# jts/nanopolish

Hardware: NVIDIA H100
Metric: hmm_scored_events_per_sec (higher is better)
Workload: dtype f32

## Files before the change

### nanopolish_b200/csrc/hmm_classes.h

```cpp
#pragma once
#include <stdint.h>

#ifdef __CUDACC__
#define NPH_HD __host__ __device__ __forceinline__
#else
#define NPH_HD inline
#endif

#define NPH_NUM_WIDTHS 5
#define NPH_MAX_COLS 10
#define NPH_NUM_CLASSES (NPH_NUM_WIDTHS * NPH_MAX_COLS)
#define NPH_STEP_BUCKETS 1024
#define NPH_CHUNK_BUCKETS 8
#define NPH_KEY_BUCKETS (NPH_STEP_BUCKETS * NPH_CHUNK_BUCKETS)
#define NPH_MIN_PERIOD 40

NPH_HD uint32_t nph_class_width(int wi) { return wi >= 3 ? 32u : (4u << wi); }
NPH_HD bool nph_class_chained(int wi) { return wi == 4; }
NPH_HD int nph_class_index(int C, int wi) { return wi * NPH_MAX_COLS + (C - 1); }

NPH_HD uint32_t nph_class_steps(uint32_t K, uint32_t E, int C, uint32_t W)
{
    const uint32_t strip = W * (uint32_t)C;
    const uint32_t n_strips = (K + strip - 1) / strip;
    const uint32_t P = n_strips > 1 ? (E > (uint32_t)NPH_MIN_PERIOD ? E : (uint32_t)NPH_MIN_PERIOD) : E;
    const uint32_t last_cols = K - (n_strips - 1) * strip;
    return (n_strips - 1) * P + E + (last_cols - 1) / (uint32_t)C;
}

NPH_HD float nph_class_cost(uint32_t steps, int C, uint32_t W)
{
    return (float)steps * (46.0f + 67.0f * C) * (W * (1.0f / 32.0f));
}

NPH_HD int nph_choose_class(uint32_t K, uint32_t E, uint32_t* steps_out)
{
    float best = 3.0e38f;
    int best_cls = nph_class_index(NPH_MAX_COLS, 4);
    uint32_t best_steps = 0;
    for (int wi = 0; wi < NPH_NUM_WIDTHS; ++wi) {
        const uint32_t W = nph_class_width(wi);
        for (int C = 1; C <= NPH_MAX_COLS; ++C) {
            const bool fits = K <= W * (uint32_t)C;
            if (nph_class_chained(wi) ? fits : !fits) continue;
            const uint32_t steps = nph_class_steps(K, E, C, W);
            const float cost = nph_class_cost(steps, C, W);
            if (cost < best) { best = cost; best_cls = nph_class_index(C, wi); best_steps = steps; }
        }
    }
    *steps_out = best_steps;
    return best_cls;
}

NPH_HD uint32_t nph_key_bucket(uint32_t steps, uint32_t chunk)
{
    uint32_t b = steps < 768u ? steps : 768u + (steps - 768u) / 32u;
    if (b >= (uint32_t)NPH_STEP_BUCKETS) b = (uint32_t)NPH_STEP_BUCKETS - 1u;
    if (chunk >= (uint32_t)NPH_CHUNK_BUCKETS) chunk = (uint32_t)NPH_CHUNK_BUCKETS - 1u;
    return chunk * (uint32_t)NPH_STEP_BUCKETS + ((uint32_t)NPH_STEP_BUCKETS - 1u - b);
}
```

### nanopolish_b200/csrc/hmm_forward.cu

```cuda
#include "hmm_forward_kernel.cuh"
#include <algorithm>
#include <cmath>
#include <vector>

using namespace nph_fwd;

namespace {

__global__ void read_prologue_kernel(const DevRead* __restrict__ reads, const double* __restrict__ drift,
                                     const float* __restrict__ ev_mean, const double* __restrict__ ev_time,
                                     float* __restrict__ level, uint32_t n_reads)
{
    for (uint32_t r = blockIdx.x; r < n_reads; r += gridDim.x) {
        const DevRead rd = reads[r];
        const double dr = drift[r];
        const float* m = ev_mean + rd.event_off;
        const double* t = ev_time + rd.event_off;
        float* out = level + rd.event_off;
        const double t0 = t[0];
        for (uint32_t i = threadIdx.x; i < rd.n_events; i += blockDim.x) {
            const float time = (float)__dsub_rn(t[i], t0);
            out[i] = (float)__dsub_rn((double)m[i], __dmul_rn((double)time, dr));
        }
    }
}

}

static void scratch_layout(const nph_ctx* ctx, NphArena& a, float4** params, float** edge)
{
    const size_t warps = (size_t)ctx->sm_count * kMaxWarpsPerCta;
    for (int si = 0; si < nph_ctx::kSideStreams; ++si) {
        params[si] = a.take<float4>((size_t)ctx->max_kpad * warps);
        edge[si] = a.take<float>(3 * ((size_t)ctx->max_period + 8) * warps);
    }
}

size_t nph_hmm_scratch_bytes(const nph_ctx* ctx)
{
    float4* params[nph_ctx::kSideStreams];
    float* edge[nph_ctx::kSideStreams];
    return nph_layout_bytes([&](NphArena& a) { scratch_layout(ctx, a, params, edge); });
}

int nph_launch_read_prologue(nph_ctx* ctx)
{
    const uint32_t n = (uint32_t)ctx->n_reads;
    if (n == 0) return NPH_OK;
    int grid = (int)std::min<size_t>(n, (size_t)ctx->sm_count * 16);
    read_prologue_kernel<<<grid, 256, 0, ctx->stream>>>(ctx->d_reads.p, ctx->d_drift.p, ctx->d_ev_mean.p,
                                                        ctx->d_ev_time.p, ctx->d_level.p, n);
    NPH_CUDA(ctx, cudaGetLastError());
    return NPH_OK;
}

int nph_launch_hmm_forward(nph_ctx* ctx, float* scores_dev)
{
    FwdParams p{};
    p.level = ctx->d_level.p;
    p.reads = ctx->d_reads.p;
    p.trans = ctx->d_trans.p;
    p.models = ctx->d_models.p;
    p.ranks = ctx->d_ranks.p;
    p.jobs = ctx->d_jobs.p;
    p.logsum_g = ctx->d_logsum.p;
    p.flank = ctx->d_flank.p;
    p.scores = scores_dev ? scores_dev : ctx->d_scores.p;
    p.kpad_stride = ctx->max_kpad;
    p.edge_stride = ctx->max_period + 8;
    p.c = ctx->consts;
    p.lsum_bias = NPH_LOGSUM_SAT_ADDR_BIAS;
    p.lsum_scale = 4u;
    p.progress = (ctx->levels_inflight && ctx->level_chunk_events) ? ctx->d_progress.p : nullptr;
    p.chunk_events = (uint32_t)ctx->level_chunk_events;
    float4* params[nph_ctx::kSideStreams];
    float* edge[nph_ctx::kSideStreams];
    NphArena scratch{ctx->d_scratch.p};
    scratch_layout(ctx, scratch, params, edge);

    NPH_CUDA(ctx, cudaMemsetAsync(ctx->d_counters.p, 0, sizeof(unsigned int) * NPH_NUM_COUNTERS, ctx->stream));
    NPH_CUDA(ctx, cudaEventRecord(ctx->ev0, ctx->stream));
    NPH_CUDA(ctx, cudaEventRecord(ctx->ev_fork, ctx->stream));
    std::vector<size_t> idx;
    for (size_t ci = 0; ci < ctx->classes.size(); ++ci) if (ctx->classes[ci].count) idx.push_back(ci);
    std::sort(idx.begin(), idx.end(), [&](size_t a, size_t b) { return ctx->classes[a].cost > ctx->classes[b].cost; });
    bool used[nph_ctx::kSideStreams] = {false, false, false, false};
    int launches = 0;
    for (size_t t = 0; t < idx.size(); ++t) {
        const size_t ci = idx[t];
        const auto& cl = ctx->classes[ci];
        const int si = (int)(t % nph_ctx::kSideStreams);
        cudaStream_t st = ctx->side[si];
        if (!used[si]) { NPH_CUDA(ctx, cudaStreamWaitEvent(st, ctx->ev_fork, 0)); used[si] = true; }
        p.scratch_params = params[si];
        p.scratch_edge = edge[si];
        int rc = NPH_ERR_STATE;
        switch (cl.group_width) {
            case 4: rc = launch_width<4, false>(ctx, p, cl, (int)ci, st); break;
            case 8: rc = launch_width<8, false>(ctx, p, cl, (int)ci, st); break;
            case 16: rc = launch_width<16, false>(ctx, p, cl, (int)ci, st); break;
            case 32: rc = cl.chained ? launch_width<32, true>(ctx, p, cl, (int)ci, st) : launch_width<32, false>(ctx, p, cl, (int)ci, st); break;
        }
        if (rc != NPH_OK) return rc;
        ++launches;
    }
    for (int si = 0; si < nph_ctx::kSideStreams; ++si) {
        if (!used[si]) continue;
        NPH_CUDA(ctx, cudaEventRecord(ctx->ev_join[si], ctx->side[si]));
        NPH_CUDA(ctx, cudaStreamWaitEvent(ctx->stream, ctx->ev_join[si], 0));
    }
    NPH_CUDA(ctx, cudaEventRecord(ctx->ev1, ctx->stream));
    nph_timing_events(ctx, launches);
    return NPH_OK;
}
```

### nanopolish_b200/csrc/hmm_forward_kernel.cuh

```cuda
#pragma once
#include "nph_internal.cuh"
#include "hmm_classes.h"
#include "exact_math.cuh"
#include <math_constants.h>
#include <climits>

namespace nph_fwd {

static_assert(NPH_TBL_SMEM == NPH_LOGSUM_TBL_LEN, "the shared table must cover every index lsum_sat can form");

constexpr int kMaxWarpsPerCta = 24;
template <int C, int W> struct CtaShape { static constexpr int warps = (W == 32) ? 16 : (C <= 4 ? 24 : (C <= 6 ? 20 : 16)); };
constexpr unsigned kFull = 0xffffffffu;

struct FwdParams {
    const float* level;
    const DevRead* reads;
    const float2* trans;
    const DevModelView* models;
    const uint32_t* ranks;
    const nph_hmm_job* jobs;
    const uint32_t* order;
    uint32_t n_jobs;
    unsigned int* counter;
    const float* logsum_g;
    const float* flank;
    float* scores;
    float4* scratch_params;
    float* scratch_edge;
    uint32_t kpad_stride;
    uint32_t edge_stride;
    uint32_t lsum_bias;
    uint32_t lsum_scale;
    const uint32_t* progress;
    uint32_t chunk_events;
    HmmConsts c;
};

template <int C, int W, bool CHAIN>
__global__ void __launch_bounds__(CtaShape<C, W>::warps * 32, 1) hmm_forward_kernel(const FwdParams p)
{
    static_assert(W == 4 || W == 8 || W == 16 || W == 32, "group width");
    static_assert(!CHAIN || W == 32, "only full-warp groups chain strips");
    constexpr int G = 32 / W;
    constexpr int kWarpsPerCta = CtaShape<C, W>::warps;
    constexpr int kCtaThreads = kWarpsPerCta * 32;
    constexpr int STRIP = W * C;
    extern __shared__ float s_tbl[];
    for (int i = threadIdx.x; i < NPH_TBL_SMEM; i += kCtaThreads) s_tbl[i] = p.logsum_g[i];
    __syncthreads();
    const LogsumTable tb = make_logsum_table(s_tbl, p.lsum_bias, p.lsum_scale);

    const int lane = threadIdx.x & 31;
    const int gl = lane & (W - 1);
    const int grp = lane / W;
    const int warp_global = blockIdx.x * kWarpsPerCta + (threadIdx.x >> 5);
    float4* const my_params = p.scratch_params + (size_t)warp_global * p.kpad_stride + (W < 32 ? grp * STRIP : 0);
    float* const edge_m = p.scratch_edge + (size_t)warp_global * 3 * p.edge_stride;
    float* const edge_t = edge_m + p.edge_stride;
    float* const edge_k = edge_t + p.edge_stride;

    const float NEG = -CUDART_INF_F;
    const float lp_mk = p.c.lp_mk, lp_mb = p.c.lp_mb, lp_bb = p.c.lp_bb, lp3 = p.c.lp_bk;
    const float lp_kk = p.c.lp_kk, lp_km = p.c.lp_km;

    for (;;) {
        uint32_t base = 0;
        if (lane == 0) base = atomicAdd(p.counter, (unsigned)G);
        base = __shfl_sync(kFull, base, 0);
        if (base >= p.n_jobs) break;
        const uint32_t slot = base + grp;
        const bool has_job = slot < p.n_jobs;
        const uint32_t job_idx = p.order[has_job ? slot : base];
        const nph_hmm_job job = p.jobs[job_idx];
        const DevRead rd = p.reads[job.read];
        const float2 tr = p.trans[job.read];
        const float lp_mm_self = tr.x, lp_mm_next = tr.y;
        const DevModelView mv = p.models[job.model_id];
        if (p.progress) {
            uint32_t need = has_job ? (uint32_t)((rd.event_off + rd.n_events - 1) / p.chunk_events) + 1u : 0u;
            need = __reduce_max_sync(kFull, need);
            if (lane == 0) {
                const volatile uint32_t* pr = p.progress;
                while (*pr < need) __nanosleep(500);
            }
            __syncwarp();
        }

        const int K = (int)job.n_kmers;
        const int E = has_job ? (int)(job.event_stop > job.event_start ? job.event_stop - job.event_start
                                                                       : job.event_start - job.event_stop) + 1
                              : 0;
        const int stride = job.stride;
        const bool pre_clip = (job.flags & NPH_HAF_ALLOW_PRE_CLIP) != 0;
        const bool post_clip = (job.flags & NPH_HAF_ALLOW_POST_CLIP) != 0;
        const int n_strips = CHAIN ? (K + STRIP - 1) / STRIP : 1;
        const int kpad = n_strips * STRIP;
        const int P = n_strips > 1 ? max(E, NPH_MIN_PERIOD) : E;

        if (has_job) {
            const uint32_t* rk = p.ranks + job.rank_off;
            for (int i = gl; i < kpad; i += W) {
                float4 g = make_float4(0.f, 1.f, 0.f, 1.f);
                if (i < K) g = nph_scaled_gaussian(mv, rd, rk[i], p.c.log_inv_sqrt_2pi);
                my_params[i] = g;
            }
        }
        __syncwarp();

        const float* lv = p.level + rd.event_off;
        const long long e_first = (long long)job.event_start;

        const int last_strip = n_strips - 1;
        const int last_rel = (K - 1) - last_strip * STRIP;
        const int end_lane = last_rel / C;
        const int end_slot = last_rel % C;
        const int my_steps = has_job ? last_strip * P + E + end_lane : 0;
        const int total_steps = (W == 32) ? my_steps : __reduce_max_sync(kFull, my_steps);
        const bool any_pre_clip = __any_sync(kFull, pre_clip);

        float mu[C], sd[C], cc[C], ry[C];
        float Mp[C], Bp[C], Kp[C], Tp[C];
#pragma unroll
        for (int c = 0; c < C; ++c) { mu[c] = 0.f; sd[c] = 1.f; cc[c] = 0.f; ry[c] = 1.f; Mp[c] = NEG; Bp[c] = NEG; Kp[c] = NEG; Tp[c] = NEG; }
        if (!CHAIN && gl * C < K) {
#pragma unroll
            for (int c = 0; c < C; ++c) {
                const float4 g4 = my_params[gl * C + c];
                mu[c] = g4.x; sd[c] = g4.y; cc[c] = g4.z; ry[c] = g4.w;
            }
        }
        float Lm_prev = NEG, Lt_prev = NEG, Lk_prev = NEG;
        float lp_end = NEG;
        int r = 1 - gl;
        int s = 0;
        float x_next = 0.f;
        if (r == 1 && E >= 1) x_next = lv[e_first];
        float em_next = NEG, et_next = NEG, ek_next = NEG;
        const long long x_step = (long long)stride * (long long)sizeof(float);
        unsigned long long x_addr = (unsigned long long)(lv + e_first) + (unsigned long long)((long long)r * x_step);
        const int end_row = (gl == end_lane) ? (post_clip ? 1 : E) : INT_MAX;

        for (int g = 0; g < total_steps; ++g) {
            float Lm = __shfl_up_sync(kFull, Mp[C - 1], 1, W);
            float Lt = __shfl_up_sync(kFull, Tp[C - 1], 1, W);
            float Lk = __shfl_up_sync(kFull, Kp[C - 1], 1, W);
            if (gl == 0) { Lm = CHAIN ? em_next : NEG; Lt = CHAIN ? et_next : NEG; Lk = CHAIN ? ek_next : NEG; }

            const bool in_strip = (r >= 1) && (!CHAIN || s < n_strips);
            const int col0 = (CHAIN ? s * STRIP : 0) + gl * C;
            const bool live = in_strip && (r <= E) && (col0 < K);
            const float x = x_next;

            if (CHAIN && in_strip && r == 1) {
#pragma unroll
                for (int c = 0; c < C; ++c) { Mp[c] = NEG; Bp[c] = NEG; Kp[c] = NEG; Tp[c] = NEG; }
                Lm_prev = NEG; Lt_prev = NEG; Lk_prev = NEG;
                if (col0 < K) {
#pragma unroll
                    for (int c = 0; c < C; ++c) {
                        const float4 g4 = my_params[col0 + c];
                        mu[c] = g4.x; sd[c] = g4.y; cc[c] = g4.z; ry[c] = g4.w;
                    }
                }
            }

            {
                int rn = r + 1, sn = s;
                if (CHAIN && rn > P) { rn = 1; sn = s + 1; }
                if (rn >= 1 && rn <= E && (!CHAIN || sn < n_strips)) {
                    x_next = CHAIN ? lv[e_first + (long long)(rn - 1) * stride] : __ldca(reinterpret_cast<const float*>(x_addr));
                    if (CHAIN && gl == 0 && sn > 0) { em_next = edge_m[rn]; et_next = edge_t[rn]; ek_next = edge_k[rn]; }
                }
            }

            if (live) {
                const bool do_end = (!CHAIN || s == last_strip) && r >= end_row;

                float lm_prev = Lm_prev, lt_prev = Lt_prev, lk_prev = Lk_prev;
                float lm_cur = Lm, lt_cur = Lt, lk_cur = Lk;
                auto cell = [&](const int c, const bool with_soft) {
                    const float a = div_by_cached_rcp(__fsub_rn(x, mu[c]), sd[c], ry[c]);
                    const float em = add_neg_half_square(cc[c], a);
                    float m = __fadd_rn(lp_mm_self, Mp[c]);
                    m = lsum_sat(m, __fadd_rn(lp_mm_next, lm_prev), tb);
                    m = lsum_sat(m, Tp[c], tb);
                    m = lsum_sat(m, lt_prev, tb);
                    m = lsum_sat(m, __fadd_rn(lp_km, lk_prev), tb);
                    if (with_soft) m = lsum_sat(m, (col0 == 0 && (r == 1 || pre_clip)) ? p.flank[r - 1] : NEG, tb);
                    m = __fadd_rn(m, em);
                    const float b = lsum_sat(__fadd_rn(lp_mb, Mp[c]), __fadd_rn(lp_bb, Bp[c]), tb);
                    float kk = lsum_sat(__fadd_rn(lp_mk, lm_cur), lt_cur, tb);
                    kk = lsum_sat(kk, __fadd_rn(lp_kk, lk_cur), tb);
                    const float t = __fadd_rn(lp3, b);

                    lm_prev = Mp[c]; lt_prev = Tp[c]; lk_prev = Kp[c];
                    lm_cur = m; lt_cur = t; lk_cur = kk;
                    Mp[c] = m; Bp[c] = b; Kp[c] = kk; Tp[c] = t;
                };
                if (any_pre_clip || g == 0) cell(0, true);
                else cell(0, false);
#pragma unroll
                for (int c = 1; c < C; ++c) cell(c, false);
                Lm_prev = Lm; Lt_prev = Lt; Lk_prev = Lk;

                if (do_end) {
                    float Me = Mp[0], Be = Bp[0], Ke = Kp[0];
#pragma unroll
                    for (int c = 1; c < C; ++c) if (c == end_slot) { Me = Mp[c]; Be = Bp[c]; Ke = Kp[c]; }
                    const float post = p.flank[E - r];
                    lp_end = lsum_sat(lp_end, __fadd_rn(Me, post), tb);
                    lp_end = lsum_sat(lp_end, __fadd_rn(Be, post), tb);
                    lp_end = lsum_sat(lp_end, __fadd_rn(Ke, post), tb);
                }
                if (CHAIN && gl == W - 1 && s < last_strip) {
                    edge_m[r] = Mp[C - 1];
                    edge_t[r] = Tp[C - 1];
                    edge_k[r] = Kp[C - 1];
                }
            }

            r += 1;
            if (!CHAIN) x_addr += x_step;
            if (CHAIN && r > P) { r = 1; s += 1; }
            if (CHAIN && n_strips > 1) __syncwarp();
        }

        const float result = __shfl_sync(kFull, lp_end, (lane & ~(W - 1)) + end_lane);
        if (gl == 0 && has_job) p.scores[job_idx] = result;
        __syncwarp();
    }
}

template <int C, int W, bool CHAIN>
int launch_class(nph_ctx* ctx, const FwdParams& base, const nph_ctx::ClassLaunch& cl, int class_idx, cudaStream_t stream)
{
    FwdParams p = base;
    p.order = ctx->d_order.p + cl.first;
    p.n_jobs = (uint32_t)cl.count;
    p.counter = ctx->d_counters.p + class_idx;
    const size_t smem = sizeof(float) * NPH_TBL_SMEM;
    NPH_CUDA(ctx, cudaFuncSetAttribute(hmm_forward_kernel<C, W, CHAIN>, cudaFuncAttributeMaxDynamicSharedMemorySize, (int)smem));
    constexpr int kWarpsPerCta = CtaShape<C, W>::warps;
    int grid = ctx->sm_count;
    const size_t warps_needed = (cl.count + (32 / W) - 1) / (32 / W);
    if ((size_t)grid * kWarpsPerCta > warps_needed) grid = (int)((warps_needed + kWarpsPerCta - 1) / kWarpsPerCta);
    if (grid < 1) grid = 1;
    hmm_forward_kernel<C, W, CHAIN><<<grid, kWarpsPerCta * 32, smem, stream>>>(p);
    NPH_CUDA(ctx, cudaGetLastError());
    return NPH_OK;
}

template <int W, bool CHAIN> int launch_width(nph_ctx* ctx, const FwdParams& base, const nph_ctx::ClassLaunch& cl, int class_idx, cudaStream_t stream);

#define NPH_DEFINE_LAUNCH_WIDTH(W, CHAIN)                                                                              \
    template <> int launch_width<W, CHAIN>(nph_ctx * ctx, const FwdParams& base, const nph_ctx::ClassLaunch& cl, int class_idx, cudaStream_t stream) \
    {                                                                                                           \
        switch (cl.cols_per_lane) {                                                                             \
            case 1: return launch_class<1, W, CHAIN>(ctx, base, cl, class_idx, stream);                                       \
            case 2: return launch_class<2, W, CHAIN>(ctx, base, cl, class_idx, stream);                                       \
            case 3: return launch_class<3, W, CHAIN>(ctx, base, cl, class_idx, stream);                                       \
            case 4: return launch_class<4, W, CHAIN>(ctx, base, cl, class_idx, stream);                                       \
            case 5: return launch_class<5, W, CHAIN>(ctx, base, cl, class_idx, stream);                                       \
            case 6: return launch_class<6, W, CHAIN>(ctx, base, cl, class_idx, stream);                                       \
            case 7: return launch_class<7, W, CHAIN>(ctx, base, cl, class_idx, stream);                                       \
            case 8: return launch_class<8, W, CHAIN>(ctx, base, cl, class_idx, stream);                                       \
            case 9: return launch_class<9, W, CHAIN>(ctx, base, cl, class_idx, stream);                                       \
            case 10: return launch_class<10, W, CHAIN>(ctx, base, cl, class_idx, stream);                                     \
        }                                                                                                       \
        return NPH_ERR_STATE;                                                                                   \
    }

}
```

Baseline: 1.297 billion.

## Stream jobs back-to-back through full-width warps with a double-buffered descriptor ring

Adds a streaming path for the 32-lane non-chained classes. Each warp pipelines consecutive jobs along its wavefront: the next job's descriptor and Gaussian parameters are fetched into a two-slot shared-memory ring while the current job is still draining, so lanes start a new job as soon as they finish rather than waiting for the whole warp. The class cost model is updated to reflect the new step count (max(E+1, min period)), and its per-column coefficients are retuned. The change also adds scratch and shared-memory sizing for the ring, more per-lane state and branching inside the step loop, and dependence on the new slot-flipping logic being correct.

```diff
diff --git a/nanopolish_b200/csrc/hmm_classes.h b/nanopolish_b200/csrc/hmm_classes.h
--- a/nanopolish_b200/csrc/hmm_classes.h
+++ b/nanopolish_b200/csrc/hmm_classes.h
@@ -28,9 +28,16 @@
     return (n_strips - 1) * P + E + (last_cols - 1) / (uint32_t)C;
 }
 
+NPH_HD uint32_t nph_fwd_class_steps(uint32_t K, uint32_t E, int C, int wi)
+{
+    const uint32_t W = nph_class_width(wi);
+    if (W == 32 && !nph_class_chained(wi)) return E + 1 > (uint32_t)NPH_MIN_PERIOD ? E + 1 : (uint32_t)NPH_MIN_PERIOD;
+    return nph_class_steps(K, E, C, W);
+}
+
 NPH_HD float nph_class_cost(uint32_t steps, int C, uint32_t W)
 {
-    return (float)steps * (46.0f + 67.0f * C) * (W * (1.0f / 32.0f));
+    return (float)steps * (44.0f + 66.0f * C) * (W * (1.0f / 32.0f));
 }
 
 NPH_HD int nph_choose_class(uint32_t K, uint32_t E, uint32_t* steps_out)
@@ -43,7 +50,7 @@
         for (int C = 1; C <= NPH_MAX_COLS; ++C) {
             const bool fits = K <= W * (uint32_t)C;
             if (nph_class_chained(wi) ? fits : !fits) continue;
-            const uint32_t steps = nph_class_steps(K, E, C, W);
+            const uint32_t steps = nph_fwd_class_steps(K, E, C, wi);
             const float cost = nph_class_cost(steps, C, W);
             if (cost < best) { best = cost; best_cls = nph_class_index(C, wi); best_steps = steps; }
         }
diff --git a/nanopolish_b200/csrc/hmm_forward.cu b/nanopolish_b200/csrc/hmm_forward.cu
--- a/nanopolish_b200/csrc/hmm_forward.cu
+++ b/nanopolish_b200/csrc/hmm_forward.cu
@@ -31,7 +31,7 @@
 {
     const size_t warps = (size_t)ctx->sm_count * kMaxWarpsPerCta;
     for (int si = 0; si < nph_ctx::kSideStreams; ++si) {
-        params[si] = a.take<float4>((size_t)ctx->max_kpad * warps);
+        params[si] = a.take<float4>((size_t)ctx->max_kpad * ctx->sm_count * kParamLinesPerCta);
         edge[si] = a.take<float>(3 * ((size_t)ctx->max_period + 8) * warps);
     }
 }
diff --git a/nanopolish_b200/csrc/hmm_forward_kernel.cuh b/nanopolish_b200/csrc/hmm_forward_kernel.cuh
--- a/nanopolish_b200/csrc/hmm_forward_kernel.cuh
+++ b/nanopolish_b200/csrc/hmm_forward_kernel.cuh
@@ -4,6 +4,7 @@
 #include "exact_math.cuh"
 #include <math_constants.h>
 #include <climits>
+#include <type_traits>
 
 namespace nph_fwd {
 
@@ -37,6 +38,200 @@
     HmmConsts c;
 };
 
+struct alignas(64) StreamDesc {
+    unsigned long long x0;
+    const float4* line;
+    int x_step;
+    int E;
+    int P;
+    int K;
+    int end_lane, end_slot;
+    uint32_t flags;
+    float lp_mm_self, lp_mm_next;
+    uint32_t score_idx;
+};
+static_assert(sizeof(StreamDesc) == 64, "a lane holds the address of its job's slot and flips between the two with one XOR");
+constexpr int kStreamWarps = 16;
+constexpr int kRingOffset = (NPH_TBL_SMEM + 31) & ~31;
+constexpr size_t kStreamSmem = sizeof(float) * kRingOffset + sizeof(StreamDesc) * 2 * kStreamWarps;
+constexpr int kParamLinesPerCta = kMaxWarpsPerCta > 2 * kStreamWarps ? kMaxWarpsPerCta : 2 * kStreamWarps;
+
+struct RowConsts { float lp_mk, lp_mb, lp_bb, lp3, lp_kk, lp_km; };
+
+template <bool WITH_SOFT>
+__device__ __forceinline__ void fwd_cell(float& M, float& B, float& Kc, float& T, const float mu, const float sd, const float cc,
+                                         const float ry, const float x, const float soft, float& lm_prev, float& lt_prev,
+                                         float& lk_prev, float& lm_cur, float& lt_cur, float& lk_cur, const float lp_mm_self,
+                                         const float lp_mm_next, const RowConsts& k, const LogsumTable& tb)
+{
+    const float a = div_by_cached_rcp(__fsub_rn(x, mu), sd, ry);
+    const float em = add_neg_half_square(cc, a);
+    float m = __fadd_rn(lp_mm_self, M);
+    m = lsum_sat(m, __fadd_rn(lp_mm_next, lm_prev), tb);
+    m = lsum_sat(m, T, tb);
+    m = lsum_sat(m, lt_prev, tb);
+    m = lsum_sat(m, __fadd_rn(k.lp_km, lk_prev), tb);
+    if (WITH_SOFT) m = lsum_sat(m, soft, tb);
+    m = __fadd_rn(m, em);
+    const float b = lsum_sat(__fadd_rn(k.lp_mb, M), __fadd_rn(k.lp_bb, B), tb);
+    float kk = lsum_sat(__fadd_rn(k.lp_mk, lm_cur), lt_cur, tb);
+    kk = lsum_sat(kk, __fadd_rn(k.lp_kk, lk_cur), tb);
+    const float t = __fadd_rn(k.lp3, b);
+
+    lm_prev = M; lt_prev = T; lk_prev = Kc;
+    lm_cur = m; lt_cur = t; lk_cur = kk;
+    M = m; B = b; Kc = kk; T = t;
+}
+
+template <int C>
+__device__ __forceinline__ void forward_stream(const FwdParams& p, const LogsumTable& tb, const RowConsts& k, float* s_tbl)
+{
+    constexpr int STRIP = 32 * C;
+    const int lane = threadIdx.x & 31;
+    const int warp = threadIdx.x >> 5;
+    const float NEG = -CUDART_INF_F;
+    float4* const params = p.scratch_params + (size_t)(blockIdx.x * kStreamWarps + warp) * 2 * p.kpad_stride;
+    StreamDesc* const ring = reinterpret_cast<StreamDesc*>(s_tbl + kRingOffset) + 2 * warp;
+
+    auto prepare = [&](const int slot) -> StreamDesc {
+        __syncwarp();
+        uint32_t n = 0;
+        if (lane == 0) n = atomicAdd(p.counter, 1u);
+        n = __shfl_sync(kFull, n, 0);
+        float4* const line = params + (size_t)slot * p.kpad_stride;
+        StreamDesc d{};
+        d.P = INT_MAX;
+        d.line = line;
+        if (n < p.n_jobs) {
+            const uint32_t job_idx = p.order[n];
+            const nph_hmm_job job = p.jobs[job_idx];
+            const DevRead rd = p.reads[job.read];
+            const float2 tr = p.trans[job.read];
+            const DevModelView mv = p.models[job.model_id];
+            if (p.progress) {
+                const uint32_t need = (uint32_t)((rd.event_off + rd.n_events - 1) / p.chunk_events) + 1u;
+                if (lane == 0) {
+                    const volatile uint32_t* pr = p.progress;
+                    while (*pr < need) __nanosleep(500);
+                }
+                __syncwarp();
+            }
+            const int K = (int)job.n_kmers;
+            const uint32_t* rk = p.ranks + job.rank_off;
+            for (int i = lane; i < STRIP; i += 32) {
+                float4 g = make_float4(0.f, 1.f, 0.f, 1.f);
+                if (i < K) g = nph_scaled_gaussian(mv, rd, rk[i], p.c.log_inv_sqrt_2pi);
+                line[i] = g;
+            }
+            d.x0 = (unsigned long long)(p.level + rd.event_off + job.event_start);
+            d.x_step = job.stride * (int)sizeof(float);
+            d.E = (int)(job.event_stop > job.event_start ? job.event_stop - job.event_start : job.event_start - job.event_stop) + 1;
+            d.P = max(d.E + 1, NPH_MIN_PERIOD);
+            d.K = K;
+            d.end_lane = (K - 1) / C;
+            d.end_slot = (K - 1) % C;
+            d.flags = job.flags;
+            d.lp_mm_self = tr.x;
+            d.lp_mm_next = tr.y;
+            d.score_idx = job_idx;
+        }
+        if (lane == 0) ring[slot] = d;
+        __syncwarp();
+        return d;
+    };
+
+    StreamDesc d = prepare(0);
+    if (d.E == 0) return;
+
+    int slot = 1, r = -lane, P = 0, E_live = -32, end_row = INT_MAX;
+    float lp_mm_self = 0.f, lp_mm_next = 0.f, lp_end = NEG;
+    float mu[C], sd[C], cc[C], ry[C];
+    float Mp[C], Bp[C], Kp[C], Tp[C];
+#pragma unroll
+    for (int c = 0; c < C; ++c) { mu[c] = 0.f; sd[c] = 1.f; cc[c] = 0.f; ry[c] = 1.f; Mp[c] = NEG; Bp[c] = NEG; Kp[c] = NEG; Tp[c] = NEG; }
+    float Lm_prev = NEG, Lt_prev = NEG, Lk_prev = NEG;
+    float x_next = 0.f;
+    int x_step = 0;
+    unsigned long long x_addr = 0;
+    auto load_gaussians = [&](const float4* line) {
+        line += lane * C;
+#pragma unroll
+        for (int c = 0; c < C; ++c) {
+            const float4 g4 = line[c];
+            mu[c] = g4.x; sd[c] = g4.y; cc[c] = g4.z; ry[c] = g4.w;
+        }
+    };
+
+    auto step = [&](auto soft_tag) {
+        constexpr bool SOFT = decltype(soft_tag)::value;
+        float Lm = __shfl_up_sync(kFull, Mp[C - 1], 1);
+        float Lt = __shfl_up_sync(kFull, Tp[C - 1], 1);
+        float Lk = __shfl_up_sync(kFull, Kp[C - 1], 1);
+        if (lane == 0) { Lm = NEG; Lt = NEG; Lk = NEG; }
+        const float x = x_next;
+
+        if (r <= E_live) {
+            if (r < E_live) x_next = __ldca(reinterpret_cast<const float*>(x_addr));
+            float lm_prev = Lm_prev, lt_prev = Lt_prev, lk_prev = Lk_prev;
+            float lm_cur = Lm, lt_cur = Lt, lk_cur = Lk;
+            fwd_cell<SOFT>(Mp[0], Bp[0], Kp[0], Tp[0], mu[0], sd[0], cc[0], ry[0], x, (SOFT && lane == 0) ? p.flank[r - 1] : NEG,
+                           lm_prev, lt_prev, lk_prev, lm_cur, lt_cur, lk_cur, lp_mm_self, lp_mm_next, k, tb);
+#pragma unroll
+            for (int c = 1; c < C; ++c)
+                fwd_cell<false>(Mp[c], Bp[c], Kp[c], Tp[c], mu[c], sd[c], cc[c], ry[c], x, NEG, lm_prev, lt_prev, lk_prev,
+                                lm_cur, lt_cur, lk_cur, lp_mm_self, lp_mm_next, k, tb);
+            Lm_prev = Lm; Lt_prev = Lt; Lk_prev = Lk;
+
+            if (r >= end_row) {
+                const StreamDesc& e = ring[slot];
+                const int end_slot = e.end_slot;
+                float Me = Mp[0], Be = Bp[0], Ke = Kp[0];
+#pragma unroll
+                for (int c = 1; c < C; ++c) if (c == end_slot) { Me = Mp[c]; Be = Bp[c]; Ke = Kp[c]; }
+                const float post = p.flank[E_live - r];
+                lp_end = lsum_sat(lp_end, __fadd_rn(Me, post), tb);
+                lp_end = lsum_sat(lp_end, __fadd_rn(Be, post), tb);
+                lp_end = lsum_sat(lp_end, __fadd_rn(Ke, post), tb);
+                if (r == E_live) p.scores[e.score_idx] = lp_end;
+            }
+        } else if (r >= P) {
+            slot ^= 1;
+            const StreamDesc e = ring[slot];
+            r = 0;
+            P = e.P;
+            E_live = lane * C < e.K ? e.E : 0;
+            end_row = lane == e.end_lane ? ((e.flags & NPH_HAF_ALLOW_POST_CLIP) ? 1 : e.E) : INT_MAX;
+            lp_mm_self = e.lp_mm_self;
+            lp_mm_next = e.lp_mm_next;
+            x_step = e.x_step;
+            x_addr = e.x0;
+            if (E_live >= 1) x_next = __ldca(reinterpret_cast<const float*>(e.x0));
+            load_gaussians(e.line);
+#pragma unroll
+            for (int c = 0; c < C; ++c) { Mp[c] = NEG; Bp[c] = NEG; Kp[c] = NEG; Tp[c] = NEG; }
+            Lm_prev = NEG; Lt_prev = NEG; Lk_prev = NEG;
+            lp_end = NEG;
+        }
+
+        r += 1;
+        x_addr += (long long)x_step;
+    };
+
+    int left = 0;
+    for (;;) {
+        const bool more = d.E != 0;
+        left = max(left, more ? 1 + d.E + d.end_lane : 0);
+        const int seg = more ? d.P : left;
+        int n = seg;
+        for (int n_soft = (d.flags & NPH_HAF_ALLOW_PRE_CLIP) ? seg : min(2, seg); n_soft > 0; --n_soft, --n) step(std::true_type{});
+        for (; n > 0; --n) step(std::false_type{});
+        if (!more) break;
+        left -= seg;
+        d = prepare(__shfl_sync(kFull, slot, 0) ^ 1);
+        load_gaussians(ring[slot].line);
+    }
+}
+
 template <int C, int W, bool CHAIN>
 __global__ void __launch_bounds__(CtaShape<C, W>::warps * 32, 1) hmm_forward_kernel(const FwdParams p)
 {
@@ -50,6 +245,12 @@
     for (int i = threadIdx.x; i < NPH_TBL_SMEM; i += kCtaThreads) s_tbl[i] = p.logsum_g[i];
     __syncthreads();
     const LogsumTable tb = make_logsum_table(s_tbl, p.lsum_bias, p.lsum_scale);
+    const RowConsts k{p.c.lp_mk, p.c.lp_mb, p.c.lp_bb, p.c.lp_bk, p.c.lp_kk, p.c.lp_km};
+    if constexpr (W == 32 && !CHAIN) {
+        static_assert(kWarpsPerCta == kStreamWarps, "stream scratch is laid out for this CTA shape");
+        forward_stream<C>(p, tb, k, s_tbl);
+        return;
+    }
 
     const int lane = threadIdx.x & 31;
     const int gl = lane & (W - 1);
@@ -61,8 +262,6 @@
     float* const edge_k = edge_t + p.edge_stride;
 
     const float NEG = -CUDART_INF_F;
-    const float lp_mk = p.c.lp_mk, lp_mb = p.c.lp_mb, lp_bb = p.c.lp_bb, lp3 = p.c.lp_bk;
-    const float lp_kk = p.c.lp_kk, lp_km = p.c.lp_km;
 
     for (;;) {
         uint32_t base = 0;
@@ -180,23 +379,13 @@
                 float lm_prev = Lm_prev, lt_prev = Lt_prev, lk_prev = Lk_prev;
                 float lm_cur = Lm, lt_cur = Lt, lk_cur = Lk;
                 auto cell = [&](const int c, const bool with_soft) {
-                    const float a = div_by_cached_rcp(__fsub_rn(x, mu[c]), sd[c], ry[c]);
-                    const float em = add_neg_half_square(cc[c], a);
-                    float m = __fadd_rn(lp_mm_self, Mp[c]);
-                    m = lsum_sat(m, __fadd_rn(lp_mm_next, lm_prev), tb);
-                    m = lsum_sat(m, Tp[c], tb);
-                    m = lsum_sat(m, lt_prev, tb);
-                    m = lsum_sat(m, __fadd_rn(lp_km, lk_prev), tb);
-                    if (with_soft) m = lsum_sat(m, (col0 == 0 && (r == 1 || pre_clip)) ? p.flank[r - 1] : NEG, tb);
-                    m = __fadd_rn(m, em);
-                    const float b = lsum_sat(__fadd_rn(lp_mb, Mp[c]), __fadd_rn(lp_bb, Bp[c]), tb);
-                    float kk = lsum_sat(__fadd_rn(lp_mk, lm_cur), lt_cur, tb);
-                    kk = lsum_sat(kk, __fadd_rn(lp_kk, lk_cur), tb);
-                    const float t = __fadd_rn(lp3, b);
-
-                    lm_prev = Mp[c]; lt_prev = Tp[c]; lk_prev = Kp[c];
-                    lm_cur = m; lt_cur = t; lk_cur = kk;
-                    Mp[c] = m; Bp[c] = b; Kp[c] = kk; Tp[c] = t;
+                    if (with_soft)
+                        fwd_cell<true>(Mp[c], Bp[c], Kp[c], Tp[c], mu[c], sd[c], cc[c], ry[c], x,
+                                       (col0 == 0 && (r == 1 || pre_clip)) ? p.flank[r - 1] : NEG, lm_prev, lt_prev, lk_prev,
+                                       lm_cur, lt_cur, lk_cur, lp_mm_self, lp_mm_next, k, tb);
+                    else
+                        fwd_cell<false>(Mp[c], Bp[c], Kp[c], Tp[c], mu[c], sd[c], cc[c], ry[c], x, NEG, lm_prev, lt_prev,
+                                        lk_prev, lm_cur, lt_cur, lk_cur, lp_mm_self, lp_mm_next, k, tb);
                 };
                 if (any_pre_clip || g == 0) cell(0, true);
                 else cell(0, false);
@@ -239,7 +428,7 @@
     p.order = ctx->d_order.p + cl.first;
     p.n_jobs = (uint32_t)cl.count;
     p.counter = ctx->d_counters.p + class_idx;
-    const size_t smem = sizeof(float) * NPH_TBL_SMEM;
+    const size_t smem = (W == 32 && !CHAIN) ? kStreamSmem : sizeof(float) * NPH_TBL_SMEM;
     NPH_CUDA(ctx, cudaFuncSetAttribute(hmm_forward_kernel<C, W, CHAIN>, cudaFuncAttributeMaxDynamicSharedMemorySize, (int)smem));
     constexpr int kWarpsPerCta = CtaShape<C, W>::warps;
     int grid = ctx->sm_count;
```

New measurement: 1.330 billion, median of 6. 1.03x the previous value.
